# ctu-mrs/mrs_multirotor_simulator

Hardware: NVIDIA B200
Metric: UAV-steps/s (RK4+control+collisions) at 1M UAVs (higher is better)
Workload: dtype f64

## Files before the change

mrs_multirotor_simulator_b200/csrc/api.cu:

```cuda
#include <dlfcn.h>
#include <nccl.h>

#include <algorithm>
#include <cmath>
#include <cstdarg>
#include <cstdio>
#include <cstring>
#include <functional>
#include <map>
#include <memory>
#include <string>
#include <utility>
#include <vector>

#include "internal.h"
#include "params.h"

static thread_local char g_err[512] = "";

static int fail(int code, const char* fmt, ...) {
  va_list ap;
  va_start(ap, fmt);
  vsnprintf(g_err, sizeof(g_err), fmt, ap);
  va_end(ap);
// ... 147 lines not shown

  bool                 p2p       = false;
  double*              gbuf[2]   = {nullptr, nullptr};
  uint32_t*            d_gbox[2] = {nullptr, nullptr};
  int64_t              pass_no   = 0;
  bool                 wrote_since_pass = false;
  std::vector<int32_t> pending_geom[2];
  PeerView             pv[2]{};
  PeerView             pv_local{};
  P2PCtl               p2pctl{};
  unsigned long long*  d_flags   = nullptr;
  unsigned long long** d_peer_flags = nullptr;
  std::vector<void*>   ipc_opened;
  Mem<int, true>       h_status;

  cudaStream_t up_stream = nullptr, down_stream = nullptr;
  Mem<double>  d_up[2];
  Mem<double>  d_snap[2];
  cudaEvent_t  ev_up[2] = {nullptr, nullptr}, ev_applied[2] = {nullptr, nullptr}, ev_snap[2] = {nullptr, nullptr}, ev_down[2] = {nullptr, nullptr};
  uint64_t     n_up = 0, n_down = 0;
  Mem<int32_t> d_sub_idx;
  int64_t      n_sub = 0;

  cudaGraphExec_t coll_graph[2]     = {nullptr, nullptr};
  int             coll_graph_own[2] = {0, 0};

  bool     lists_on            = false;
  int      steps_since_pass    = 0;
  bool     positions_touched   = true;
  int      rebuild_own         = 0;
  int64_t  list_passes         = 0;
  bool     list_graph_failed   = false;
  int64_t  rebuilds_counted    = 0;
  Mem<uint32_t, true> h_one;
  cudaGraphExec_t tick_graph[2] = {nullptr, nullptr};
  double   tick_dt = 0.0;
  int      tick_k = 0, tick_mode = -2, tick_own[2] = {0, 0};
  uint64_t tick_pset = ~0ull;
  uint32_t tick_opts = 0;
  bool     tick_failed = false;

  int64_t n_steps = 0, n_passes = 0, n_launches = 0;
  int     step_info[4] = {0, 0, 0, 0};
};

static void drop_collision_graphs(mrsb_sim* h) {
  for (int k = 0; k < 2; k++) {
    if (h->coll_graph[k]) cudaGraphExecDestroy(h->coll_graph[k]);
    h->coll_graph[k] = nullptr;
    if (h->tick_graph[k]) cudaGraphExecDestroy(h->tick_graph[k]);
    h->tick_graph[k] = nullptr;
  }
}

static std::string set_key(const ParamSet& s) {
  return std::string(reinterpret_cast<const char*>(&s), sizeof(ParamSet));
}

static int intern_set(mrsb_sim* h, const ParamSet& s) {
  const std::string key = set_key(s);
  auto              it  = h->set_index.find(key);
  if (it != h->set_index.end()) return it->second;
  const int id = int(h->sets.size());
  h->sets.push_back(s);
  h->set_index[key] = id;
  h->params_dirty   = true;
// ... 22 lines not shown
  s.cp.att_kp = cp.att_kp, s.cp.att_kd = cp.att_kd, s.cp.att_ki = cp.att_ki, s.cp.att_max_rate_roll_pitch = cp.att_max_rate_roll_pitch,
  s.cp.att_max_rate_yaw = cp.att_max_rate_yaw;
  s.cp.vel_kp = cp.vel_kp, s.cp.vel_kd = cp.vel_kd, s.cp.vel_ki = cp.vel_ki, s.cp.vel_max_acceleration = cp.vel_max_acceleration;
  s.cp.pos_kp = cp.pos_kp, s.cp.pos_kd = cp.pos_kd, s.cp.pos_ki = cp.pos_ki, s.cp.pos_max_velocity = cp.pos_max_velocity;
  return s;
}

static int collect_param_sets(mrsb_sim* h) {
  const int n_sets = int(h->sets.size());
  if (n_sets <= 32) return MRSB_OK;
  std::vector<int> refs(size_t(n_sets), 0);
  for (int32_t id : h->pset_host) refs[size_t(id)]++;
  int live = 0;
  for (int r : refs) live += r > 0;
  if (2 * live > n_sets) return MRSB_OK;
  std::vector<int>      remap(size_t(n_sets), -1);
  std::vector<ParamSet> kept;
  kept.reserve(size_t(live));
  h->set_index.clear();
  for (int k = 0; k < n_sets; k++) {
    if (!refs[size_t(k)]) continue;
    remap[size_t(k)] = int(kept.size());
    h->set_index[set_key(h->sets[size_t(k)])] = int(kept.size());
    kept.push_back(h->sets[size_t(k)]);
  }
  h->sets.swap(kept);
  h->tick_pset = ~0ull;
  for (int32_t& id : h->pset_host) id = remap[size_t(id)];
  CU(cudaMemcpyAsync(h->d_pset, h->pset_host.data(), sizeof(int32_t) * h->pset_host.size(), cudaMemcpyHostToDevice, h->stream));
  CU(cudaStreamSynchronize(h->stream));
  return MRSB_OK;
}

static int flush_params(mrsb_sim* h) {
  if (!h->params_dirty) return MRSB_OK;
  int rc = collect_param_sets(h);
  if (rc) return rc;
  const int    n_sets = int(h->sets.size());
  const size_t cap    = size_t(std::max(16, 2 * n_sets));
  rc                  = h->d_params.grow(size_t(n_sets), cap, h->stream);
  if (rc) return rc;
  if (h->ds.params != h->d_params.get()) {
    h->ds.params = h->d_params.get();
    drop_collision_graphs(h);
  }
  rc = h->d_takeoff0.grow(size_t(n_sets), cap, h->stream);
  if (rc) return rc;
  std::vector<DevParams> host(n_sets);
  std::vector<uint8_t>   takeoff0(size_t(n_sets), 0);
  for (int k = 0; k < n_sets; k++) {
    mrsb_derive(h->sets[k].mp, h->sets[k].cp, &host[k]);
    takeoff0[size_t(k)] = h->sets[k].mp.takeoff_patch_enabled != 0;
  }
  CU(cudaMemcpyAsync(h->d_params.get(), host.data(), sizeof(DevParams) * n_sets, cudaMemcpyHostToDevice, h->stream));
  CU(cudaMemcpyAsync(h->d_takeoff0.get(), takeoff0.data(), size_t(n_sets), cudaMemcpyHostToDevice, h->stream));
  CU(cudaStreamSynchronize(h->stream));
  h->filt_dt = -1.0;
  for (mrsb_sim::Bucket& b : h->buckets) {
    int nm = -1, ps = -2;
    for (int64_t k = 0; k < b.count; k++) {
      const int64_t e  = h->inv_host.empty() ? b.slot0 + k : h->inv_host[size_t(b.slot0 + k)];
      const int     id = h->pset_host[size_t(h->ds.shard_begin + e)];
      const int     m  = h->sets[size_t(id)].mp.n_motors;
      if (nm == -1) nm = m;
      if (nm != m) nm = 0;
      if (ps == -2) ps = id;
      if (ps != id) ps = -1;
      if (nm == 0 && ps == -1) break;
    }
    b.nm   = nm > 0 ? nm : 0;
    b.pset = ps >= 0 ? ps : -1;
    if (b.pset >= 0) b.params = host[size_t(b.pset)];
  }
  h->params_dirty = false;
  return MRSB_OK;
}

static int ensure_filt(mrsb_sim* h, double dt) {
  if (h->filt_dt == dt) return MRSB_OK;
  h->n_launches += launch_prep_params(h->d_params.get(), int(h->sets.size()), dt, h->stream);
  for (mrsb_sim::Bucket& b : h->buckets)
    if (b.pset >= 0) CU(cudaMemcpyAsync(&b.params.filt, &h->d_params.get()[b.pset].filt, sizeof(double), cudaMemcpyDeviceToHost, h->stream));
  CU(cudaStreamSynchronize(h->stream));
  h->filt_dt = dt;
  for (int k = 0; k < 2; k++) {
    if (h->tick_graph[k]) cudaGraphExecDestroy(h->tick_graph[k]);
    h->tick_graph[k] = nullptr;
  }
  return MRSB_OK;
}

static int ensure_stage(mrsb_sim* h, size_t bytes) {
  return h->d_stage.grow(bytes, std::max<size_t>(bytes, 1 << 16), h->stream);
}

static int stage_idx(mrsb_sim* h, int64_t n, const int32_t* idx, const int32_t** out) {
  *out = nullptr;
  if (n < 0 || n > h->ds.n && !idx) return fail(MRSB_ERR_INVALID, "n=%lld outside 0..%lld", (long long)n, (long long)h->ds.n);
  if (!idx || n == 0) return MRSB_OK;
  for (int64_t k = 0; k < n; k++)
    if (idx[k] < 0 || idx[k] >= h->ds.n) return fail(MRSB_ERR_INVALID, "idx[%lld]=%d outside 0..%lld", (long long)k, idx[k], (long long)h->ds.n - 1);
  int rc = h->d_idx.grow(size_t(n), std::max<size_t>(size_t(n), 1024), h->stream);
  if (rc) return rc;
  CU(cudaMemcpyAsync(h->d_idx.get(), idx, sizeof(int32_t) * n, cudaMemcpyHostToDevice, h->stream));
  *out = h->d_idx.get();
  return MRSB_OK;
}

// ... 139 lines not shown
      memo[key] = id;
      const mrsb_model_params &a = h->sets[size_t(old)].mp, &b = h->sets[size_t(id)].mp;
      if (a.arm_length != b.arm_length || a.prop_radius != b.prop_radius || a.mass != b.mass) geometry = true;
    }
    ids[size_t(k)]                                 = id;
    h->pset_host[size_t(h->ds.shard_begin + i)] = id;
  }
  if (geometry && h->ds.n_global > h->ds.n && !h->p2p) {
    for (int64_t k = n - 1; k >= 0; k--) h->pset_host[size_t(h->ds.shard_begin + (idx ? idx[k] : k))] = olds[size_t(k)];
    return fail(MRSB_ERR_STATE, "arm length / propeller radius / mass of a sharded handle can only change while its peers read them from this "
                                "GPU (exchange mode 2, mrsb_comm_init_nccl with peer access)");
  }
  h->params_dirty = true;
  rc              = ensure_stage(h, sizeof(int32_t) * size_t(n));
  if (rc) return rc;
  CU(cudaMemcpyAsync(h->d_stage.get(), ids.data(), sizeof(int32_t) * size_t(n), cudaMemcpyHostToDevice, h->stream));
  h->n_launches += launch_set_pset(h->d_pset, n, d_idx, h->ds.shard_begin, reinterpret_cast<const int32_t*>(h->d_stage.get()), h->stream);
  CU(cudaStreamSynchronize(h->stream));
  if (geometry) {
    rc = flush_params(h);
    if (rc) return rc;
    rc = stage_idx(h, n, idx, &d_idx);
    if (rc) return rc;
    rc = geometry_changed(h, n, idx, d_idx);
    if (rc) return rc;
    CU(cudaStreamSynchronize(h->stream));
  }
  return MRSB_OK;
}

static void set_collision_geometry(mrsb_sim* h, bool lists) {
  DevGrid& g  = h->grid;
  h->lists_on = lists;
  double cell = lists ? 6.0 : 4.0;
  if (const char* e = getenv("MRSB_COLLISION_CELL")) cell = std::max(3.5, atof(e));
  g.inv_cell = 1.0 / cell;
  g.reach    = 0.5 * cell;
  const double r_list = g.reach * (1.0 - 1e-6);
  g.list_r2  = r_list * r_list;
  g.skin     = (r_list - 1.7320508075688775) * (1.0 - 1e-6);
  h->ds.disp_max       = lists ? &g.ctl->disp_max_bits : nullptr;
  h->positions_touched = true;
}

static void make_local_view(mrsb_sim* h) {
  PeerView& v = h->pv_local;
  v           = PeerView{};
  v.n_ranks   = 1;
  v.rank      = 0;
  v.begin[0]  = 0;
  v.begin[1]  = h->ds.n_global;
  v.pos[0]    = h->ds.gpos;
  v.geom[0]   = h->d_geom[0];
}

static int setup_p2p(mrsb_sim* h) {
  const int    G     = h->n_ranks;
  const size_t ng    = size_t(h->ds.n_global);
  h->gbuf[0]         = h->ds.gpos;
  int rc             = dalloc(h, &h->gbuf[1], 3 * ng);
  if (rc) return rc;
  CU(cudaMemcpy(h->gbuf[1], h->gbuf[0], sizeof(double) * 3 * ng, cudaMemcpyDeviceToDevice));
  rc = dalloc(h, &h->d_geom[1], 4 * ng);
  if (rc) return rc;
  CU(cudaMemcpy(h->d_geom[1], h->d_geom[0], sizeof(double) * 4 * ng, cudaMemcpyDeviceToDevice));
  for (int k = 0; k < 2; k++) {
    rc = dalloc(h, &h->d_gbox[k], 6 * size_t(h->ds.ld / 32 + 1));
    if (rc) return rc;
  }
  rc = dalloc(h, &h->d_flags, 3 * size_t(G));
  if (rc) return rc;
  rc = h->h_status.alloc(1);
  if (rc) return rc;
// ... 275 lines not shown
    DevGrid&     g  = h->grid;
    const size_t ng = size_t(std::max<int64_t>(s.n_global, 1));
    const size_t own    = size_t(std::max<int64_t>(s.n, 1));
    const size_t expect = std::max<size_t>(std::min(ng, own + own / 4 + 4096), 512);
    uint32_t     bits   = 10;
    while (2 * (size_t(1) << bits) < 3 * expect && bits < 30) bits++;
    g.bits      = bits;
    g.n_buckets = 1u << bits;
    g.pair_cap   = int64_t(std::max<size_t>(4096, 4 * size_t(std::max<int64_t>(s.n, 1))));
    g.scan_tiles = scan_tiles_for(int64_t(g.n_buckets) + 3);
    g.halo_cap   = std::max<int64_t>(s.n_global - s.n, 1);
    rc = dalloc(h, &g.bucket, ng);
    if (!rc) rc = dalloc(h, &g.rank, ng);
    if (!rc) rc = dalloc(h, &g.count, size_t(g.n_buckets) + 4);
    if (!rc) rc = dalloc(h, &g.begin, size_t(g.n_buckets) + 4);
    if (!rc) rc = dalloc(h, &g.aabb, 6);
    if (!rc) rc = dalloc(h, &g.rec, 2 * ng);
    if (!rc) rc = h->pairs.grow(2 * size_t(g.pair_cap), 2 * size_t(g.pair_cap), h->stream);
    if (!rc) rc = dalloc(h, &g.counters, 4);
    if (!rc) rc = dalloc(h, &g.scan_state, size_t(g.scan_tiles) + size_t(scan_tiles_for(s.n)) + 2);
    if (!rc && s.n_global > s.n) rc = dalloc(h, &g.halo_rec, size_t(g.halo_cap));
    if (!rc && s.n_global > s.n) rc = dalloc(h, &g.halo_bucket, size_t(g.halo_cap));
    if (!rc && s.n_global > s.n) rc = dalloc(h, &g.halo_rank, size_t(g.halo_cap));
    if (!rc) rc = dalloc(h, &g.halo_n, 2);
    if (!rc && s.n_global > s.n) rc = dalloc(h, &g.halo_work, size_t(g.halo_cap / 32 + MRSB_MAX_RANKS + 1));
    if (!rc && getenv("MRSB_TIMELINE")) rc = dalloc(h, &g.tl, size_t(MRSB_TL_TICKS) * 8);
    if (!rc) rc = dalloc(h, &g.ctl, 1);
    if (!rc) rc = h->h_one.alloc(2);
    if (rc) return rc;
    g.pairs       = h->pairs.get();
    g.halo_work_n = g.halo_n + 1;
    h->h_one.get()[0] = 1u;
    h->h_one.get()[1] = 0xFFFFFFFFu;
    if (s.n > 0 && !getenv("MRSB_NO_NEIGHBOUR_LISTS")) {
      g.nl_ld = s.ld;
      rc      = dalloc(h, &g.nl_count, size_t(g.nl_ld));
      if (!rc) rc = dalloc(h, &g.nl_items, size_t(MRSB_NL_CAP) * size_t(g.nl_ld));
      if (!rc) rc = dalloc(h, &g.nl_active, size_t(g.nl_ld));
      if (!rc) rc = dalloc(h, &g.act_items, size_t(MRSB_NL_CAP) * size_t(g.nl_ld));
      if (rc) return rc;
    }
    set_collision_geometry(h, g.nl_count != nullptr && s.n_global == s.n);
  }
  make_local_view(h);
  h->shard_begin_of = {s.shard_begin};
  h->shard_count_of = {s.n};
  CU(cudaStreamSynchronize(h->stream));
  *out = guard.release();
  return MRSB_OK;
}

int mrsb_sync(mrsb_handle h) {
  GUARD(h);
  CU(cudaStreamSynchronize(h->stream));
  if (h->up_stream) CU(cudaStreamSynchronize(h->up_stream));
  if (h->down_stream) CU(cudaStreamSynchronize(h->down_stream));
  return MRSB_OK;
}

static int ensure_pipeline(mrsb_sim* h) {
  if (h->d_snap[1].get()) return MRSB_OK;
  for (cudaStream_t* s : {&h->up_stream, &h->down_stream})
    if (!*s) CU(cudaStreamCreateWithFlags(s, cudaStreamNonBlocking));
  const size_t snap = 3 * size_t(std::max<int64_t>(h->ds.n, 1));
  for (int k = 0; k < 2; k++) {
    for (cudaEvent_t* e : {&h->ev_up[k], &h->ev_applied[k], &h->ev_snap[k], &h->ev_down[k]})
      if (!*e) CU(cudaEventCreateWithFlags(e, cudaEventDisableTiming));
    int rc = h->d_snap[k].grow(snap, snap, h->down_stream);
    if (rc) return rc;
  }
  return MRSB_OK;
}
// ... 288 lines not shown
    if (cudaStreamGetCaptureInfo_v2(h->stream, &status, nullptr, &graph, nullptr, nullptr) != cudaSuccess || !graph) break;
    if (with_step) *own_fixed += launch_step_buckets(h, dt, k_sub);
    ok = capture_list_pass(h, v, graph, &side, own_fixed, own_rebuild);
  } while (false);
  cudaGraph_t captured = nullptr;
  const bool  ended    = cudaStreamEndCapture(h->stream, &captured) == cudaSuccess && captured;
  if (ok && ended && cudaGraphInstantiate(&exec, captured, 0) != cudaSuccess) exec = nullptr;
  if (captured) cudaGraphDestroy(captured);
  if (side) cudaStreamDestroy(side);
  cudaGetLastError();
  return exec;
}

static int before_list_pass(mrsb_sim* h) {
  if (h->positions_touched || h->steps_since_pass != 1)
    CU(cudaMemcpyAsync(&h->grid.ctl->force, h->h_one.get(), sizeof(uint32_t), cudaMemcpyHostToDevice, h->stream));
  h->positions_touched = false;
  h->steps_since_pass  = 0;
  h->list_passes++;
  return MRSB_OK;
}

static int after_pass(mrsb_sim* h) {
  h->n_passes++;
  if (h->p2p) {
    h->pass_no++;
    const int w         = write_buf(h);
    h->ds.gpos          = h->gbuf[w];
    h->ds.gbox          = h->d_gbox[w];
    h->ds.geom          = h->d_geom[w];
    h->wrote_since_pass = false;
    int rc              = apply_pending_geom(h, w);
    if (rc) return rc;
  }
  CU(cudaGetLastError());
  return MRSB_OK;
}

static int collide_local(mrsb_sim* h) {
  if (h->p2p && !h->wrote_since_pass) {
    h->n_launches += launch_publish_positions(h->ds, h->stream);
    h->wrote_since_pass = true;
  }
  const PassView v = pass_view(h);
  const int      k = v.k;
  if (h->lists_on) {
    int rc = before_list_pass(h);
    if (rc) return rc;
    if (!h->coll_graph[k] && !h->list_graph_failed && !getenv("MRSB_NO_GRAPH")) {
      h->coll_graph[k]     = build_pass_graph(h, v, false, 0.0, 0, &h->coll_graph_own[k], &h->rebuild_own);
      h->list_graph_failed = h->coll_graph[k] == nullptr;
    }
    if (h->coll_graph[k]) {
      CU(cudaGraphLaunch(h->coll_graph[k], h->stream));
      h->n_launches += h->coll_graph_own[k];
    } else {
      h->n_launches += launch_collide_decide(h->grid, h->p2pctl, 1, cudaGraphConditionalHandle{}, 0, h->stream);
      h->rebuild_own = launch_collide_rebuild(v.s, h->grid, *v.pv, h->stream);
      h->rebuild_own += launch_collide_check(v.s, h->grid, *v.pv, h->coll_crash, h->coll_rebounce, 0, h->stream);
    }
    return after_pass(h);
  }
  if (!h->coll_graph[k] && !getenv("MRSB_NO_GRAPH")) {
    cudaGraph_t graph = nullptr;
    if (cudaStreamBeginCapture(h->stream, cudaStreamCaptureModeThreadLocal) == cudaSuccess) {
      const int own = launch_collide(v.s, h->grid, *v.pv, h->p2pctl, h->coll_crash, h->coll_rebounce, h->stream);
// ... 582 lines not shown
  GUARD(h);
  if (!out4) return fail(MRSB_ERR_INVALID, "null output");
  for (int k = 0; k < 4; k++) out4[k] = h->step_info[k];
  return MRSB_OK;
}

int mrsb_get_timeline(mrsb_handle h, uint64_t* out, int64_t max_passes, int64_t* n_passes) {
  GUARD(h);
  CU(cudaStreamSynchronize(h->stream));
  if (n_passes) *n_passes = 0;
  if (!h->grid.tl) return fail(MRSB_ERR_STATE, "no timeline: set MRSB_TIMELINE=1 before mrsb_create");
  NlCtl ctl{};
  CU(cudaMemcpy(&ctl, h->grid.ctl, sizeof(ctl), cudaMemcpyDeviceToHost));
  const int64_t have = std::min<int64_t>(std::min<int64_t>(int64_t(ctl.n_passes), MRSB_TL_TICKS), max_passes);
  if (n_passes) *n_passes = have;
  if (!out || have <= 0) return MRSB_OK;
  std::vector<uint64_t> all(size_t(MRSB_TL_TICKS) * 8);
  CU(cudaMemcpy(all.data(), h->grid.tl, sizeof(uint64_t) * all.size(), cudaMemcpyDeviceToHost));
  for (int64_t k = 0; k < have; k++) {
    const uint64_t pass = ctl.n_passes - uint64_t(have) + uint64_t(k);
    std::memcpy(out + 8 * k, all.data() + (pass % MRSB_TL_TICKS) * 8, sizeof(uint64_t) * 8);
  }
  return MRSB_OK;
}

int mrsb_get_collision_info(mrsb_handle h, double* out8) {
  GUARD(h);
  CU(cudaStreamSynchronize(h->stream));
  NlCtl ctl{};
  if (h->lists_on) CU(cudaMemcpy(&ctl, h->grid.ctl, sizeof(ctl), cudaMemcpyDeviceToHost));
  out8[0] = 1.0 / h->grid.inv_cell;
  out8[1] = h->lists_on ? 1.0 : 0.0;
  out8[2] = h->lists_on ? std::sqrt(h->grid.list_r2) : 0.0;
  out8[3] = h->lists_on ? h->grid.skin : 0.0;
  out8[4] = double(ctl.n_passes);
  out8[5] = double(ctl.n_rebuilds);
  out8[6] = double(ctl.n_crowded);
  out8[7] = double(h->grid.n_buckets);
  return MRSB_OK;
}

int mrsb_nccl_unique_id(void* out128) {
  int rc = load_nccl();
  if (rc) return rc;
  ncclUniqueId id;
  NC(g_nccl.GetUniqueId(&id));
  std::memcpy(out128, &id, sizeof(id));
  return MRSB_OK;
}

int mrsb_comm_init_nccl(mrsb_handle h, int32_t n_ranks, int32_t rank, const void* unique_id128) {
  GUARD(h);
  int rc = load_nccl();
  if (rc) return rc;
  if (n_ranks < 1 || rank < 0 || rank >= n_ranks) return fail(MRSB_ERR_INVALID, "bad rank %d of %d", rank, n_ranks);
  ncclUniqueId id;
  std::memcpy(&id, unique_id128, sizeof(id));
  NC(g_nccl.CommInitRank(&h->comm, n_ranks, id, rank));
  h->n_ranks = n_ranks;
  h->rank    = rank;
  Mem<int64_t> d_tab;
  rc = d_tab.alloc(2 * size_t(n_ranks));
  if (rc) return rc;
  const int64_t mine[2] = {h->ds.shard_begin, h->ds.n};
  CU(cudaMemcpyAsync(d_tab.get() + 2 * rank, mine, sizeof(mine), cudaMemcpyHostToDevice, h->stream));
  NC(g_nccl.AllGather(d_tab.get() + 2 * rank, d_tab.get(), 2, ncclInt64, h->comm, h->stream));
  std::vector<int64_t> tab(2 * size_t(n_ranks));
// ... 61 lines not shown
```

mrs_multirotor_simulator_b200/csrc/collide.cu:

```cuda
#include <algorithm>

#include "internal.h"

namespace {

#define DEV __device__ __forceinline__

#define NL_LIVE 0x80000000u
#define NL_CROWDED 0x40000000u

DEV unsigned long long now_ns() {
  unsigned long long t;
  asm volatile("mov.u64 %0, %globaltimer;" : "=l"(t));
  return t;
}
DEV void stamp(const DevGrid& g, int slot, unsigned long long value) {
  if (g.tl) g.tl[((g.ctl->n_passes - 1ull) % MRSB_TL_TICKS) * 8 + slot] = value;
}

DEV int cell_of(double v, double inv_cell) {
  return __double2int_rd(__dmul_rn(v, inv_cell));
}

DEV uint32_t row_hash(int cy, int cz) {
// ... 493 lines not shown
  const uint32_t full  = 0xffffffffu;
  const int      lane  = threadIdx.x & 31;
  const int      k     = threadIdx.x & 3;
  const int64_t  n_rec = int64_t(g.begin[g.n_buckets]);
  const uint32_t quad  = 0xFu << (lane & ~3);
  const uint32_t below = quad & ((1u << lane) - 1u);
  const uint32_t mask  = g.n_buckets - 1;
  const bool     write_all = g.ctl->n_passes <= g.ctl->write_all_until;
  for (int64_t p0 = int64_t(blockIdx.x) * 32; p0 < n_rec; p0 += int64_t(gridDim.x) * 32) {
    const int64_t p   = p0 + (threadIdx.x >> 2);
    const bool    has = p < n_rec;
    double4       q   = make_double4(0.0, 0.0, 0.0, 0.0);
    if (has) q = g.rec[p];
    const int64_t gi   = __double_as_longlong(q.w);
    const int64_t li   = gi - s.shard_begin;
    const bool    mine = has && li >= 0 && li < s.n;
    const int cx0 = cell_of(q.x - g.reach, g.inv_cell), cy0 = cell_of(q.y - g.reach, g.inv_cell), cz0 = cell_of(q.z - g.reach, g.inv_cell);
    uint32_t  lo = 0, len = 0;
    if (mine) {
      const uint32_t b0 = (row_hash(cy0 + (k & 1), cz0 + (k >> 1)) + uint32_t(cx0)) & mask;
      lo                = g.begin[b0];
      len               = g.begin[b0 + 2] - lo;
    }
    const int      qb  = lane & ~3;
    const uint32_t lo0 = __shfl_sync(full, lo, qb), lo1 = __shfl_sync(full, lo, qb + 1), lo2 = __shfl_sync(full, lo, qb + 2), lo3 = __shfl_sync(full, lo, qb + 3);
    const uint32_t c1  = __shfl_sync(full, len, qb);
    const uint32_t c2  = c1 + __shfl_sync(full, len, qb + 1);
    const uint32_t c3  = c2 + __shfl_sync(full, len, qb + 2);
    const uint32_t tot = c3 + __shfl_sync(full, len, qb + 3);
    auto where = [&](uint32_t c, int& row) -> uint32_t {
      row = int(c >= c1) + int(c >= c2) + int(c >= c3);
      return row == 0 ? lo0 + c : (row == 1 ? lo1 + (c - c1) : (row == 2 ? lo2 + (c - c2) : lo3 + (c - c3)));
    };
    uint32_t cnt = 0;
    for (uint32_t c = uint32_t(k); __any_sync(full, c < tot); c += 8) {
      double4 r[2];
      int     row[2] = {0, 0};
#pragma unroll
      for (int u = 0; u < 2; u++)
        if (c + 4 * u < tot) r[u] = g.rec[where(c + 4 * u, row[u])];
#pragma unroll
      for (int u = 0; u < 2; u++) {
        bool    take = false;
        int32_t gj   = 0;
        if (c + 4 * u < tot) {
          gj = int32_t(__double_as_longlong(r[u].w));
          if (int64_t(gj) != gi && nf_dist2(q.x, q.y, q.z, r[u].x, r[u].y, r[u].z) < g.list_r2 && cell_of(r[u].y, g.inv_cell) == cy0 + (row[u] & 1) &&
              cell_of(r[u].z, g.inv_cell) == cz0 + (row[u] >> 1))
            take = true;
        }
        const uint32_t bal = __ballot_sync(full, take) & quad;
        if (take) {
          const uint32_t slot = cnt + __popc(bal & below);
          if (slot < MRSB_NL_CAP) g.nl_items[int64_t(slot) * g.nl_ld + li] = gj;
        }
        cnt += __popc(bal);
      }
    }
    __syncwarp();
    const bool lead = mine && k == 0;
    if (lead) {
      uint32_t live = g.nl_count[li] & NL_LIVE;
      if (cnt == 0u && (live || write_all)) {
        const int64_t sl            = slot_of(s, li);
        s.fext[tix(F3_ROWS, 0, sl)] = 0.0;
        s.fext[tix(F3_ROWS, 1, sl)] = 0.0;
        s.fext[tix(F3_ROWS, 2, sl)] = 0.0;
        live                        = 0u;
      }
      if (cnt > MRSB_NL_CAP) {
        g.nl_items[li] = int32_t(uint32_t(p));
        g.nl_count[li] = NL_CROWDED | live;
        atomicAdd(&g.ctl->n_crowded, 1u);
      } else {
        g.nl_count[li] = cnt | live;
      }
    }
  }
}

__global__ void __launch_bounds__(256) compact_kernel(DevGrid g, const uint32_t* __restrict__ slot, int64_t n) {
  const int64_t li = int64_t(blockIdx.x) * blockDim.x + threadIdx.x;
  if (li >= n) return;
  const uint32_t word = g.nl_count[li];
  const bool     work = (word & 0x7FFFFFFFu) != 0u;
  if (work) {
    const uint32_t k   = slot[li];
    g.nl_active[k]     = make_uint2(uint32_t(li), word);
    const uint32_t cnt = (word & NL_CROWDED) ? 1u : (word & ~(NL_LIVE | NL_CROWDED));
    for (uint32_t c = 0; c < cnt; c++) g.act_items[int64_t(c) * g.nl_ld + k] = g.nl_items[int64_t(c) * g.nl_ld + li];
  }
  if (li == n - 1) g.ctl->n_active = slot[li] + (work ? 1u : 0u);
}

DEV void check_crowded(const DevState& s, const DevGrid& g, int crash_mode, double rebounce, int64_t gi, uint32_t rec_index, PairAcc& acc) {
  const double4 qb = g.rec[rec_index];
  const Stencil st = stencil_of(g, qb.x, qb.y, qb.z);
  const double* qp = s.gpos + 3 * gi;
  const double  qx = qp[0], qy = qp[1], qz = qp[2];
  auto in_ball = [&](const double4& r, int k) {
    const int64_t gj = __double_as_longlong(r.w);
    if (gj == gi) return false;
    if (cell_of(r.y, g.inv_cell) != st.rcy[k] || cell_of(r.z, g.inv_cell) != st.rcz[k]) return false;
    double rx, ry, rz;
    load_pos(s, gj, rx, ry, rz);
    return nf_dist2(qx, qy, qz, rx, ry, rz) < 3.0;
  };
  const Geom Gi      = load_geom(s, gi);
  auto       process = [&](int64_t gj) {
    double rx, ry, rz;
    load_pos(s, gj, rx, ry, rz);
    process_pair(s, g, crash_mode, rebounce, gi, qx, qy, qz, Gi, gj, rx, ry, rz, acc);
  };
  int     n_ball = 0;
  int64_t h0 = 0, h1 = 0;
  for (int k = 0; k < 4; k++)
    for (uint32_t t = st.lo[k]; t < st.hi[k]; t++) {
      const double4 r = g.rec[t];
      if (!in_ball(r, k)) continue;
      if (n_ball == 0) h0 = __double_as_longlong(r.w);
      if (n_ball == 1) h1 = __double_as_longlong(r.w);
      n_ball++;
    }
  if (n_ball <= 2) {
    if (n_ball >= 1) process(h0);
    if (n_ball == 2) process(h1);
    return;
  }
  int64_t last = -1;
  for (int c = 0; c < n_ball; c++) {
    int64_t best = INT64_MAX;
    for (int k = 0; k < 4; k++)
      for (uint32_t t = st.lo[k]; t < st.hi[k]; t++) {
        const double4 r  = g.rec[t];
        const int64_t gj = __double_as_longlong(r.w);
        if (gj <= last || gj >= best || !in_ball(r, k)) continue;
        best = gj;
      }
    if (best == INT64_MAX) break;
    process(best);
    last = best;
  }
}

DEV void check_one(const DevState& s, const DevGrid& g, int crash_mode, double rebounce, uint32_t k, int64_t li, uint32_t word, const int32_t* first4) {
  const uint32_t cnt  = word & ~(NL_LIVE | NL_CROWDED);
  const bool     live = (word & NL_LIVE) || g.ctl->n_passes <= g.ctl->write_all_until;
  PairAcc acc;
  if (word & NL_CROWDED) {
    check_crowded(s, g, crash_mode, rebounce, li + s.shard_begin, uint32_t(first4[0]), acc);
  } else if (cnt) {
    const int64_t gi = li + s.shard_begin;
    const double* qp = s.gpos + 3 * gi;
    const double  qx = qp[0], qy = qp[1], qz = qp[2];
    uint32_t      hits = 0;
    for (uint32_t base = 0; base < cnt; base += 4) {
      int32_t gj[4];
      double  r[4][3];
#pragma unroll
      for (int u = 0; u < 4; u++) gj[u] = base + u < cnt ? (base == 0 ? first4[u] : g.act_items[int64_t(base + u) * g.nl_ld + k]) : -1;
#pragma unroll
      for (int u = 0; u < 4; u++) load_pos(s, int64_t(max(gj[u], 0)), r[u][0], r[u][1], r[u][2]);
#pragma unroll
      for (int u = 0; u < 4; u++)
        if (gj[u] >= 0 && nf_dist2(qx, qy, qz, r[u][0], r[u][1], r[u][2]) < 3.0) hits |= 1u << (base + u);
    }
    if (hits) {
      const Geom Gi      = load_geom(s, gi);
      auto       process = [&](uint32_t c) {
        const int64_t gj = g.act_items[int64_t(c) * g.nl_ld + k];
        double        rx, ry, rz;
        load_pos(s, gj, rx, ry, rz);
        process_pair(s, g, crash_mode, rebounce, gi, qx, qy, qz, Gi, gj, rx, ry, rz, acc);
      };
      if (__popc(hits) <= 2) {
        while (hits) {
          process(uint32_t(__ffs(int(hits)) - 1));
          hits &= hits - 1;
        }
      } else {
        int64_t last = -1;
        while (hits) {
          int64_t  best = INT64_MAX;
          uint32_t bc   = 0;
          for (uint32_t m = hits; m; m &= m - 1) {
            const uint32_t c  = uint32_t(__ffs(int(m)) - 1);
            const int64_t  gj = g.act_items[int64_t(c) * g.nl_ld + k];
            if (gj > last && gj < best) best = gj, bc = c;
          }
          if (best == INT64_MAX) break;
          process(bc);
          last = best;
          hits &= ~(1u << bc);
        }
      }
    }
  }
  const bool nz = nonzero(acc);
  if (live || nz) store_result(s, li, acc);
  else if (acc.crashed_me) s.flags[slot_of(s, li)] |= FLAG_CRASHED;
  if (nz != bool(word & NL_LIVE)) {
    const uint32_t nw = (word & ~NL_LIVE) | (nz ? NL_LIVE : 0u);
    g.nl_count[li]    = nw;
    g.nl_active[k].y  = nw;
  }
}

#ifndef MRSB_CHECK_THREADS
#define MRSB_CHECK_THREADS 256
#define MRSB_CHECK_MINB 4
#endif
__global__ void __launch_bounds__(MRSB_CHECK_THREADS, MRSB_CHECK_MINB) check_kernel(DevState s, DevGrid g, int crash_mode, double rebounce, int skip_if_rebuild) {
  if (skip_if_rebuild && g.ctl->rebuild) return;
  if (blockIdx.x == 0 && threadIdx.x == 0) stamp(g, 4, now_ns());
  const uint32_t n_active = g.ctl->n_active;
  for (uint32_t k = blockIdx.x * blockDim.x + threadIdx.x; k < n_active; k += gridDim.x * blockDim.x) {
    const uint2 e = g.nl_active[k];
    int32_t     first4[4];
#pragma unroll
    for (int u = 0; u < 4; u++) first4[u] = g.act_items[int64_t(u) * g.nl_ld + k];
    check_one(s, g, crash_mode, rebounce, k, int64_t(e.x), e.y, first4);
  }
}

__global__ void __launch_bounds__(32) decide_kernel(NlCtl* __restrict__ c, unsigned long long* __restrict__ pair_counter, double skin, int always,
                                                    cudaGraphConditionalHandle handle, int has_handle, P2PCtl p, unsigned long long* tl) {
  const uint32_t full = 0xffffffffu;
  const int      lane = threadIdx.x;
  unsigned long long* row = tl ? tl + (c->n_passes % MRSB_TL_TICKS) * 8 : nullptr;
  if (row && lane == 0) row[0] = now_ns();
  uint32_t                 bits  = c->disp_max_bits;
  const double             D_old = c->D_total;
  const uint32_t           force = c->force, valid = c->valid;
  const unsigned long long n_rebuilds = c->n_rebuilds, n_passes = c->n_passes;
  if (p.n_ranks > 1) {
    const unsigned long long epoch = c->epoch + 1ull;
    const int                slot  = int(epoch & 1ull);
    const bool               peer  = lane < p.n_ranks && lane != p.rank;
    volatile unsigned long long* theirs = peer ? p.peer_flags[lane] : nullptr;
    if (peer) theirs[p.n_ranks + 2 * p.rank + slot] = (unsigned long long)(always ? 0xFFFFFFFFu : bits);
    __threadfence_system();
    if (peer) theirs[p.rank] = epoch;
    if (row && lane == 0) row[1] = now_ns();
    uint32_t got = 0u;
    if (peer) {
      volatile const unsigned long long* mine = p.flags;
      const long long                    t0   = clock64();
      bool                               ok   = true;
      while (mine[lane] < epoch) {
        if (clock64() - t0 > p.budget) {
          *p.status = 1;
          ok        = false;
          break;
        }
        __nanosleep(32);
      }
      __threadfence_system();
      got = ok ? uint32_t(mine[p.n_ranks + 2 * lane + slot]) : 0xFFFFFFFFu;
    }
    bits = max(bits, __reduce_max_sync(full, got));
    if (lane == 0) c->epoch = epoch;
  }
  if (lane != 0) return;
  if (row) row[2] = now_ns();
  const double d       = __dsqrt_ru(double(__uint_as_float(bits)));
  double       D       = __dadd_ru(D_old, d);
  const bool   rebuild = always || force || !valid || !(__dmul_ru(2.0, D) <= skin);
  if (has_handle) cudaGraphSetConditional(handle, rebuild ? 1u : 0u);
  *pair_counter    = 0ull;
  c->disp_max_bits = 0u;
  if (rebuild) {
    D            = 0.0;
    c->force     = 0u;
    c->valid     = 1u;
    c->n_crowded = 0u;
    c->n_active  = 0u;
    c->n_rebuilds = n_rebuilds + 1ull;
  }
  if (row) row[5] = rebuild ? 1ull : 0ull;
  c->D_total  = D;
  c->rebuild  = rebuild ? 1u : 0u;
  c->n_passes = n_passes + 1ull;
}

}

int scan_tiles_for(int64_t n_items) {
  return int((n_items + SCAN_TILE - 1) / SCAN_TILE);
}

static int launch_table(const DevState& s, const DevGrid& g, const PeerView& pv, cudaStream_t stream) {
  const int      T      = 256;
  const bool     pull   = pv.n_ranks > 1;
  const int      filter = !pull && s.n_global > s.n;
  const int64_t  j0     = pull ? s.shard_begin : 0;
  const int64_t  cnt    = pull ? s.n : s.n_global;
  const unsigned nb     = unsigned((cnt + T - 1) / T);
  const int64_t  n_scan = int64_t(g.n_buckets) + 3;
  int            own    = 0;
  cudaMemsetAsync(g.count, 0, sizeof(uint32_t) * size_t(n_scan), stream);
  cudaMemsetAsync(g.scan_state, 0, sizeof(unsigned long long) * size_t(2 + g.scan_tiles + scan_tiles_for(s.n)), stream);
  if (filter) {
    box_reset_kernel<<<1, 32, 0, stream>>>(g.aabb);
    if (s.n > 0) box_kernel<<<unsigned(std::min<int64_t>((s.n + T - 1) / T, 296)), T, 0, stream>>>(s.gpos, s.shard_begin, s.n, g.aabb);
    own += 2;
  }
  if (pull) {
    cudaMemsetAsync(g.halo_n, 0, 2 * sizeof(uint32_t), stream);
    box_reset_kernel<<<1, 32, 0, stream>>>(g.aabb);
    const int64_t n_groups = (s.n + 31) / 32;
    if (n_groups > 0) box_from_groups_kernel<<<unsigned(std::min<int64_t>((n_groups + 255) / 256, 148)), 256, 0, stream>>>(s.gbox, n_groups, g.aabb);
    own += 2;
  }
// ... 10 lines not shown
      halo_fetch_kernel<<<148 * 2, T, 0, stream>>>(s, g, pv, g.n_buckets - 1);
      own += 2;
    }
  }
  scan_kernel<false><<<unsigned(g.scan_tiles), 256, 0, stream>>>(g.count, g.begin, n_scan, g.scan_state);
  own += 1;
  if (cnt > 0) {
    scatter_kernel<<<nb, T, 0, stream>>>(s.gpos, j0, cnt, g.bucket, g.rank, g.begin, g.n_buckets, g.rec);
    own += 1;
  }
  if (pull) {
    scatter_halo_kernel<<<unsigned(std::min<int64_t>((g.halo_cap + T - 1) / T, 148 * 4)), T, 0, stream>>>(g);
    own += 1;
  }
  return own;
}

int launch_collide(const DevState& s, const DevGrid& g, const PeerView& pv, const P2PCtl& p2p, int crash_mode, double rebounce, cudaStream_t stream) {
  const int64_t n = s.n_global;
  if (n <= 0) return 0;
  int own = 0;
  if (p2p.n_ranks > 1) {
    own += launch_collide_decide(g, p2p, 1, cudaGraphConditionalHandle{}, 0, stream);
  } else {
    cudaMemsetAsync(g.counters, 0, sizeof(unsigned long long), stream);
  }
  own += launch_table(s, g, pv, stream);
  const int64_t n_rec_max = pv.n_ranks > 1 ? s.n + g.halo_cap : n;
  collide_kernel<<<unsigned((n_rec_max + 127) / 128), 128, 0, stream>>>(s, g, crash_mode, rebounce);
  return own + 1;
}

int launch_collide_decide(const DevGrid& g, const P2PCtl& p2p, int always, cudaGraphConditionalHandle handle, int has_handle, cudaStream_t stream) {
  decide_kernel<<<1, 32, 0, stream>>>(g.ctl, g.counters, g.skin, always, handle, has_handle, p2p, g.tl);
  return 1;
}
int launch_collide_rebuild(const DevState& s, const DevGrid& g, const PeerView& pv, cudaStream_t stream) {
  if (s.n_global <= 0) return 0;
  const int     own       = launch_table(s, g, pv, stream);
  const int64_t n_rec_max = pv.n_ranks > 1 ? s.n + g.halo_cap : s.n_global;
  build_lists_kernel<<<unsigned(std::max<int64_t>(1, std::min<int64_t>((n_rec_max + 31) / 32, 148 * 16))), 128, 0, stream>>>(s, g);
  if (s.n <= 0) return own + 1;
  scan_kernel<true><<<unsigned(scan_tiles_for(s.n)), 256, 0, stream>>>(g.nl_count, g.rank, s.n, g.scan_state + 1 + g.scan_tiles);
  compact_kernel<<<unsigned((s.n + 255) / 256), 256, 0, stream>>>(g, g.rank, s.n);
  return own + 3;
}
int launch_collide_check(const DevState& s, const DevGrid& g, const PeerView& pv, int crash_mode, double rebounce, int beside_rebuild, cudaStream_t stream) {
  if (s.n <= 0) return 0;
  int own = 0;
  if (pv.n_ranks > 1 && beside_rebuild) {
    refresh_halo_kernel<<<unsigned(std::max<int64_t>(1, std::min<int64_t>((g.halo_cap + 63) / 64, 148 * 2))), 64, 0, stream>>>(s, g, pv);
    own += 1;
  }
  check_kernel<<<unsigned(std::min<int64_t>((s.n + MRSB_CHECK_THREADS - 1) / MRSB_CHECK_THREADS, 148 * MRSB_CHECK_MINB)), MRSB_CHECK_THREADS, 0, stream>>>(s, g, crash_mode, rebounce,
                                                                                                                                                       beside_rebuild);
  return own + 1;
}
```

mrs_multirotor_simulator_b200/csrc/internal.h:

```cpp
#pragma once
#include <cuda_runtime.h>
#include <stdint.h>

#include "../../include/mrsb.h"

#define MRSB_NM MRSB_MAX_MOTORS
#define MRSB_TILE 128

static __host__ __device__ __forceinline__ int64_t tix(int rows, int row, int64_t i) {
  return ((i >> 7) * rows + row) * MRSB_TILE + (i & (MRSB_TILE - 1));
}
#define ST_ROWS 18
#define VPREV_ROWS 3
#define F3_ROWS 3

#define FLAG_CRASHED 1u
#define FLAG_TAKEOFF 2u
#define FLAG_VPREV 4u
#define FLAG_HAD_INPUT 256u
#define FLAG_FF_VEL_HDG_RATE 16u
#define FLAG_FF_VEL_HDG 32u
#define FLAG_FF_ACC_HDG_RATE 64u
#define FLAG_FF_ACC_HDG 128u

// ... 58 lines not shown
#define STEP_OPT_IMU 1u
#define STEP_OPT_GPOS 2u
#define STEP_OPT_NEED_INPUT 4u

#define MRSB_MAX_RANKS 16
struct PeerView {
  int32_t         n_ranks, rank;
  int64_t         begin[MRSB_MAX_RANKS + 1];
  const double*   pos[MRSB_MAX_RANKS];
  const uint32_t* box[MRSB_MAX_RANKS];
  const double*   geom[MRSB_MAX_RANKS];
};

struct P2PCtl {
  unsigned long long* const* peer_flags;
  unsigned long long*        flags;
  int32_t                    n_ranks, rank;
  int*                       status;
  long long                  budget;
};

#define MRSB_NL_CAP 8
#define MRSB_TL_TICKS 4096
struct NlCtl {
  uint32_t disp_max_bits;
  uint32_t force;
  uint32_t valid;
  uint32_t n_active;
  uint32_t n_crowded;
  uint32_t rebuild;
  double   D_total;
  unsigned long long n_rebuilds, n_passes, epoch ;
  unsigned long long write_all_until;
};

struct DevGrid {
  uint32_t  n_buckets;
  uint32_t  bits;
  double    inv_cell;
  double    reach;
  double    list_r2;
  double    skin;
  uint32_t* nl_count;
  int32_t*  nl_items;
  int64_t   nl_ld;
  uint2*    nl_active;
  int32_t*  act_items;
  NlCtl*    ctl;
  uint32_t* bucket;
  uint32_t* rank;
  uint32_t* count;
  uint32_t* begin;
  double4*  rec;
  unsigned long long* aabb;
  unsigned long long* scan_state;
  int32_t   scan_tiles;
  double4*  halo_rec;
  uint32_t* halo_bucket, *halo_rank;
  uint32_t* halo_n;
  uint32_t* halo_work;
  uint32_t* halo_work_n;
  int64_t   halo_cap;
  unsigned long long* tl;
  int32_t*  pairs;
  int64_t   pair_cap;
  unsigned long long* counters;
};

int launch_step(const DevState& s, const DevParams* uniform_params, double dt, int k_substeps, int uniform_mode, int uniform_nm, bool any_moment,
                cudaStream_t stream, int* info);
int launch_prep_params(DevParams* params, int n_sets, double dt, cudaStream_t stream);
int launch_collide(const DevState& s, const DevGrid& g, const PeerView& pv, const P2PCtl& p2p, int crash_mode, double rebounce, cudaStream_t stream);
int launch_collide_decide(const DevGrid& g, const P2PCtl& p2p, int always, cudaGraphConditionalHandle handle, int has_handle, cudaStream_t stream);
int launch_collide_rebuild(const DevState& s, const DevGrid& g, const PeerView& pv, cudaStream_t stream);
int launch_collide_check(const DevState& s, const DevGrid& g, const PeerView& pv, int crash_mode, double rebounce, int beside_rebuild, cudaStream_t stream);
int scan_tiles_for(int64_t n_items);
int launch_publish_positions(const DevState& s, cudaStream_t stream);

int launch_scatter_input(const DevState& s, int mode, int64_t n, const int32_t* idx_dev, const double* payload_dev, int stride, cudaStream_t stream);
int launch_scatter_rows(double* dst, int rows_total, int row0, int rows, int64_t n, const int32_t* idx_dev, const double* payload_dev, int stride,
// ... 22 lines not shown
```

Before: 6.336 billion.

## Derive contact radius from params, shrink list cell, skip far neighbour checks

Computes a contact radius from the largest arm length plus prop radius across parameter sets instead of always using sqrt(3). This tightens the neighbour-list skin so rebuilds happen less often. The list cell size drops from 6 to 5 to shorten the candidate lists. Each list entry now stores the nearest-neighbour distance at build time, so the check pass can skip agents whose accumulated displacement cannot yet bring them into contact. The cost is extra state, radius exchange in the multi-GPU decide handshake, and more reliance on conservative floating-point rounding.

Measured after the change: 6.537 billion (median of 6 runs). 1.03x the previous value.

```diff
diff --git a/mrs_multirotor_simulator_b200/csrc/api.cu b/mrs_multirotor_simulator_b200/csrc/api.cu
--- a/mrs_multirotor_simulator_b200/csrc/api.cu
+++ b/mrs_multirotor_simulator_b200/csrc/api.cu
@@ -203,6 +203,8 @@
   int64_t  list_passes         = 0;
   bool     list_graph_failed   = false;
   int64_t  rebuilds_counted    = 0;
+  double   r_contact           = 1.7320508075688775;
+  double   r_contact_next      = -1.0;
   Mem<uint32_t, true> h_one;
   cudaGraphExec_t tick_graph[2] = {nullptr, nullptr};
   double   tick_dt = 0.0;
@@ -291,6 +293,34 @@
   return MRSB_OK;
 }
 
+static double contact_radius(const std::vector<ParamSet>& sets) {
+  const double sqrt3 = 1.7320508075688775;
+  double       c     = 0.0;
+  for (const ParamSet& s : sets) {
+    const double a = s.mp.arm_length, p = s.mp.prop_radius;
+    if (!(a >= 0.0 && p >= 0.0 && std::isfinite(a) && std::isfinite(p))) return sqrt3;
+    c = std::max(c, a + p);
+  }
+  if (!(2.0 * c < 3.0)) return sqrt3;
+  return std::min(sqrt3, std::sqrt(2.0 * c) * (1.0 + 1e-9));
+}
+
+static int write_contact_bound(mrsb_sim* h) {
+  CU(cudaMemcpyAsync(&h->grid.ctl->r_contact, &h->r_contact, sizeof(double), cudaMemcpyHostToDevice, h->stream));
+  CU(cudaStreamSynchronize(h->stream));
+  return MRSB_OK;
+}
+static int set_contact_bound(mrsb_sim* h, double v) {
+  if (h->p2p && v < h->r_contact) {
+    h->r_contact_next = v;
+    return MRSB_OK;
+  }
+  h->r_contact_next = -1.0;
+  if (v == h->r_contact) return MRSB_OK;
+  h->r_contact = v;
+  return h->grid.ctl ? write_contact_bound(h) : MRSB_OK;
+}
+
 static int flush_params(mrsb_sim* h) {
   if (!h->params_dirty) return MRSB_OK;
   int rc = collect_param_sets(h);
@@ -332,7 +362,7 @@
     if (b.pset >= 0) b.params = host[size_t(b.pset)];
   }
   h->params_dirty = false;
-  return MRSB_OK;
+  return set_contact_bound(h, contact_radius(h->sets));
 }
 
 static int ensure_filt(mrsb_sim* h, double dt) {
@@ -538,13 +568,12 @@
 static void set_collision_geometry(mrsb_sim* h, bool lists) {
   DevGrid& g  = h->grid;
   h->lists_on = lists;
-  double cell = lists ? 6.0 : 4.0;
+  double cell = lists ? 5.0 : 4.0;
   if (const char* e = getenv("MRSB_COLLISION_CELL")) cell = std::max(3.5, atof(e));
   g.inv_cell = 1.0 / cell;
   g.reach    = 0.5 * cell;
-  const double r_list = g.reach * (1.0 - 1e-6);
-  g.list_r2  = r_list * r_list;
-  g.skin     = (r_list - 1.7320508075688775) * (1.0 - 1e-6);
+  g.r_list   = g.reach * (1.0 - 1e-6);
+  g.list_r2  = g.r_list * g.r_list;
   h->ds.disp_max       = lists ? &g.ctl->disp_max_bits : nullptr;
   h->positions_touched = true;
 }
@@ -886,12 +915,16 @@
     g.halo_work_n = g.halo_n + 1;
     h->h_one.get()[0] = 1u;
     h->h_one.get()[1] = 0xFFFFFFFFu;
+    rc                = write_contact_bound(h);
+    if (rc) return rc;
     if (s.n > 0 && !getenv("MRSB_NO_NEIGHBOUR_LISTS")) {
       g.nl_ld = s.ld;
       rc      = dalloc(h, &g.nl_count, size_t(g.nl_ld));
       if (!rc) rc = dalloc(h, &g.nl_items, size_t(MRSB_NL_CAP) * size_t(g.nl_ld));
       if (!rc) rc = dalloc(h, &g.nl_active, size_t(g.nl_ld));
       if (!rc) rc = dalloc(h, &g.act_items, size_t(MRSB_NL_CAP) * size_t(g.nl_ld));
+      if (!rc) rc = dalloc(h, &g.nl_near, size_t(g.nl_ld));
+      if (!rc) rc = dalloc(h, &g.act_near, size_t(g.nl_ld));
       if (rc) return rc;
     }
     set_collision_geometry(h, g.nl_count != nullptr && s.n_global == s.n);
@@ -1246,6 +1279,12 @@
     h->wrote_since_pass = false;
     int rc              = apply_pending_geom(h, w);
     if (rc) return rc;
+    if (h->r_contact_next >= 0.0) {
+      h->r_contact      = h->r_contact_next;
+      h->r_contact_next = -1.0;
+      rc                = write_contact_bound(h);
+      if (rc) return rc;
+    }
   }
   CU(cudaGetLastError());
   return MRSB_OK;
@@ -1894,7 +1933,7 @@
   out8[0] = 1.0 / h->grid.inv_cell;
   out8[1] = h->lists_on ? 1.0 : 0.0;
   out8[2] = h->lists_on ? std::sqrt(h->grid.list_r2) : 0.0;
-  out8[3] = h->lists_on ? h->grid.skin : 0.0;
+  out8[3] = !h->lists_on ? 0.0 : ctl.n_passes ? ctl.skin : (h->grid.r_list - h->r_contact) * (1.0 - 1e-6);
   out8[4] = double(ctl.n_passes);
   out8[5] = double(ctl.n_rebuilds);
   out8[6] = double(ctl.n_crowded);
diff --git a/mrs_multirotor_simulator_b200/csrc/collide.cu b/mrs_multirotor_simulator_b200/csrc/collide.cu
--- a/mrs_multirotor_simulator_b200/csrc/collide.cu
+++ b/mrs_multirotor_simulator_b200/csrc/collide.cu
@@ -549,7 +549,8 @@
       row = int(c >= c1) + int(c >= c2) + int(c >= c3);
       return row == 0 ? lo0 + c : (row == 1 ? lo1 + (c - c1) : (row == 2 ? lo2 + (c - c2) : lo3 + (c - c3)));
     };
-    uint32_t cnt = 0;
+    uint32_t cnt   = 0;
+    double   near2 = INFINITY;
     for (uint32_t c = uint32_t(k); __any_sync(full, c < tot); c += 8) {
       double4 r[2];
       int     row[2] = {0, 0};
@@ -561,10 +562,13 @@
         bool    take = false;
         int32_t gj   = 0;
         if (c + 4 * u < tot) {
-          gj = int32_t(__double_as_longlong(r[u].w));
-          if (int64_t(gj) != gi && nf_dist2(q.x, q.y, q.z, r[u].x, r[u].y, r[u].z) < g.list_r2 && cell_of(r[u].y, g.inv_cell) == cy0 + (row[u] & 1) &&
-              cell_of(r[u].z, g.inv_cell) == cz0 + (row[u] >> 1))
-            take = true;
+          gj              = int32_t(__double_as_longlong(r[u].w));
+          const double d2 = nf_dist2(q.x, q.y, q.z, r[u].x, r[u].y, r[u].z);
+          if (int64_t(gj) != gi && d2 < g.list_r2 && cell_of(r[u].y, g.inv_cell) == cy0 + (row[u] & 1) &&
+              cell_of(r[u].z, g.inv_cell) == cz0 + (row[u] >> 1)) {
+            take  = true;
+            near2 = fmin(near2, d2);
+          }
         }
         const uint32_t bal = __ballot_sync(full, take) & quad;
         if (take) {
@@ -575,8 +579,11 @@
       }
     }
     __syncwarp();
+    near2           = fmin(near2, __shfl_xor_sync(full, near2, 1));
+    near2           = fmin(near2, __shfl_xor_sync(full, near2, 2));
     const bool lead = mine && k == 0;
     if (lead) {
+      g.nl_near[li] = cnt > MRSB_NL_CAP ? 0.0f : __double2float_rd(__dsqrt_rd(near2));
       uint32_t live = g.nl_count[li] & NL_LIVE;
       if (cnt == 0u && (live || write_all)) {
         const int64_t sl            = slot_of(s, li);
@@ -604,6 +611,7 @@
   if (work) {
     const uint32_t k   = slot[li];
     g.nl_active[k]     = make_uint2(uint32_t(li), word);
+    g.act_near[k]      = g.nl_near[li];
     const uint32_t cnt = (word & NL_CROWDED) ? 1u : (word & ~(NL_LIVE | NL_CROWDED));
     for (uint32_t c = 0; c < cnt; c++) g.act_items[int64_t(c) * g.nl_ld + k] = g.nl_items[int64_t(c) * g.nl_ld + li];
   }
@@ -660,11 +668,13 @@
   }
 }
 
-DEV void check_one(const DevState& s, const DevGrid& g, int crash_mode, double rebounce, uint32_t k, int64_t li, uint32_t word, const int32_t* first4) {
+DEV void check_one(const DevState& s, const DevGrid& g, int crash_mode, double rebounce, uint32_t k, int64_t li, uint32_t word, const int32_t* first4,
+                   bool reach_now) {
   const uint32_t cnt  = word & ~(NL_LIVE | NL_CROWDED);
   const bool     live = (word & NL_LIVE) || g.ctl->n_passes <= g.ctl->write_all_until;
   PairAcc acc;
-  if (word & NL_CROWDED) {
+  if (!reach_now) {
+  } else if (word & NL_CROWDED) {
     check_crowded(s, g, crash_mode, rebounce, li + s.shard_begin, uint32_t(first4[0]), acc);
   } else if (cnt) {
     const int64_t gi = li + s.shard_begin;
@@ -731,22 +741,26 @@
   if (skip_if_rebuild && g.ctl->rebuild) return;
   if (blockIdx.x == 0 && threadIdx.x == 0) stamp(g, 4, now_ns());
   const uint32_t n_active = g.ctl->n_active;
+  const double   closed   = __dmul_ru(2.0, g.ctl->D_total), r_c = g.ctl->r_pass;
   for (uint32_t k = blockIdx.x * blockDim.x + threadIdx.x; k < n_active; k += gridDim.x * blockDim.x) {
-    const uint2 e = g.nl_active[k];
+    const uint2 e    = g.nl_active[k];
+    const float near = g.act_near[k];
     int32_t     first4[4];
 #pragma unroll
     for (int u = 0; u < 4; u++) first4[u] = g.act_items[int64_t(u) * g.nl_ld + k];
-    check_one(s, g, crash_mode, rebounce, k, int64_t(e.x), e.y, first4);
-  }
-}
-
-__global__ void __launch_bounds__(32) decide_kernel(NlCtl* __restrict__ c, unsigned long long* __restrict__ pair_counter, double skin, int always,
+    const bool out = closed < __dmul_rn(__dsub_rn(double(near), r_c), 1.0 - 1e-6);
+    check_one(s, g, crash_mode, rebounce, k, int64_t(e.x), e.y, first4, !out);
+  }
+}
+
+__global__ void __launch_bounds__(32) decide_kernel(NlCtl* __restrict__ c, unsigned long long* __restrict__ pair_counter, double r_list, int always,
                                                     cudaGraphConditionalHandle handle, int has_handle, P2PCtl p, unsigned long long* tl) {
   const uint32_t full = 0xffffffffu;
   const int      lane = threadIdx.x;
   unsigned long long* row = tl ? tl + (c->n_passes % MRSB_TL_TICKS) * 8 : nullptr;
   if (row && lane == 0) row[0] = now_ns();
   uint32_t                 bits  = c->disp_max_bits;
+  double                   r_c   = c->r_contact;
   const double             D_old = c->D_total;
   const uint32_t           force = c->force, valid = c->valid;
   const unsigned long long n_rebuilds = c->n_rebuilds, n_passes = c->n_passes;
@@ -755,11 +769,12 @@
     const int                slot  = int(epoch & 1ull);
     const bool               peer  = lane < p.n_ranks && lane != p.rank;
     volatile unsigned long long* theirs = peer ? p.peer_flags[lane] : nullptr;
-    if (peer) theirs[p.n_ranks + 2 * p.rank + slot] = (unsigned long long)(always ? 0xFFFFFFFFu : bits);
+    const unsigned long long rc_bits = (unsigned long long)__float_as_uint(__double2float_ru(r_c)) << 32;
+    if (peer) theirs[p.n_ranks + 2 * p.rank + slot] = rc_bits | (unsigned long long)(always ? 0xFFFFFFFFu : bits);
     __threadfence_system();
     if (peer) theirs[p.rank] = epoch;
     if (row && lane == 0) row[1] = now_ns();
-    uint32_t got = 0u;
+    unsigned long long got = 0ull;
     if (peer) {
       volatile const unsigned long long* mine = p.flags;
       const long long                    t0   = clock64();
@@ -773,15 +788,17 @@
         __nanosleep(32);
       }
       __threadfence_system();
-      got = ok ? uint32_t(mine[p.n_ranks + 2 * lane + slot]) : 0xFFFFFFFFu;
-    }
-    bits = max(bits, __reduce_max_sync(full, got));
+      got = ok ? mine[p.n_ranks + 2 * lane + slot] : 0xFFFFFFFFull;
+    }
+    bits = max(bits, __reduce_max_sync(full, uint32_t(got)));
+    r_c = double(__uint_as_float(max(uint32_t(rc_bits >> 32), __reduce_max_sync(full, uint32_t(got >> 32)))));
     if (lane == 0) c->epoch = epoch;
   }
   if (lane != 0) return;
   if (row) row[2] = now_ns();
   const double d       = __dsqrt_ru(double(__uint_as_float(bits)));
   double       D       = __dadd_ru(D_old, d);
+  const double skin    = __dmul_rn(__dsub_rn(r_list, r_c), 1.0 - 1e-6);
   const bool   rebuild = always || force || !valid || !(__dmul_ru(2.0, D) <= skin);
   if (has_handle) cudaGraphSetConditional(handle, rebuild ? 1u : 0u);
   *pair_counter    = 0ull;
@@ -796,6 +813,8 @@
   }
   if (row) row[5] = rebuild ? 1ull : 0ull;
   c->D_total  = D;
+  c->skin     = skin;
+  c->r_pass   = r_c;
   c->rebuild  = rebuild ? 1u : 0u;
   c->n_passes = n_passes + 1ull;
 }
@@ -872,7 +891,7 @@
 }
 
 int launch_collide_decide(const DevGrid& g, const P2PCtl& p2p, int always, cudaGraphConditionalHandle handle, int has_handle, cudaStream_t stream) {
-  decide_kernel<<<1, 32, 0, stream>>>(g.ctl, g.counters, g.skin, always, handle, has_handle, p2p, g.tl);
+  decide_kernel<<<1, 32, 0, stream>>>(g.ctl, g.counters, g.r_list, always, handle, has_handle, p2p, g.tl);
   return 1;
 }
 int launch_collide_rebuild(const DevState& s, const DevGrid& g, const PeerView& pv, cudaStream_t stream) {
diff --git a/mrs_multirotor_simulator_b200/csrc/internal.h b/mrs_multirotor_simulator_b200/csrc/internal.h
--- a/mrs_multirotor_simulator_b200/csrc/internal.h
+++ b/mrs_multirotor_simulator_b200/csrc/internal.h
@@ -114,6 +114,9 @@
   double   D_total;
   unsigned long long n_rebuilds, n_passes, epoch ;
   unsigned long long write_all_until;
+  double r_contact;
+  double skin;
+  double r_pass;
 };
 
 struct DevGrid {
@@ -121,13 +124,15 @@
   uint32_t  bits;
   double    inv_cell;
   double    reach;
+  double    r_list;
   double    list_r2;
-  double    skin;
   uint32_t* nl_count;
   int32_t*  nl_items;
   int64_t   nl_ld;
   uint2*    nl_active;
   int32_t*  act_items;
+  float*    nl_near;
+  float*    act_near;
   NlCtl*    ctl;
   uint32_t* bucket;
   uint32_t* rank;
```
